# smehra34/Video-Stylization-with-NCA

Hardware: AMD Instinct MI355X
Metric: NCA cell-updates/sec (B*H*W*steps/s) at 256^2 C=16 (higher is better)
Workload: dtype f32; 1 GPU; BASELINE configs[1]: ConditionedNCA grow loop, B=8 C=16 256x256, 64 NCA steps per bench step, fp32 forward; B_per_gpu=8, C=16, H=256, W=256, nca_steps_per_bench_step=64, hidden=64, mask_rng=in-kernel philox4x32-10, parallelism=pool-shard x1 (no data-path collective)

## Files before the change

### video-stylization-with-nca_amd/csrc/nca_capi.hip

```cpp
#include "../../include/ncahip.h"

#include <cstdarg>
#include <cstdio>

#include "nca_kernels.h"

namespace {

constexpr int kMaxC = 16, kMaxCCondFwd = 32, kMaxCCondFwdBf16 = 20, kMaxCDynca = 32, kMaxFc = 128, kMaxFcFwd = 1024, kMaxHidden = 64, kMaxCond = 4;

thread_local char g_err[512] = "";

int fail(int code, const char* fmt, ...) {
    va_list ap;
    va_start(ap, fmt);
    vsnprintf(g_err, sizeof(g_err), fmt, ap);
    va_end(ap);
    return code;
}

int hip_result(hipError_t e, const char* what) {
    if (e == hipSuccess) return 0;
    snprintf(g_err, sizeof(g_err), "%s: %s", what, hipGetErrorString(e));
    return (int)e;
// ... 52 lines not shown
    std::atomic<int> state{0};
    unsigned* host = nullptr;
    unsigned* dev = nullptr;
};
ErrWord g_errw[kNcaMaxDevices];
ErrWord& errw() {
    ErrWord& w = g_errw[nca_device_index()];
    if (w.state.load(std::memory_order_acquire) == 0) {
        static std::atomic_flag lock = ATOMIC_FLAG_INIT;
        while (lock.test_and_set(std::memory_order_acquire)) {}
        if (w.state.load(std::memory_order_relaxed) == 0) {
            void *h = nullptr, *d = nullptr;
            int st = 2;
            if (hipHostMalloc(&h, 64, hipHostMallocMapped) == hipSuccess && hipHostGetDevicePointer(&d, h, 0) == hipSuccess) {
                *(volatile unsigned*)h = 0u;
                w.host = (unsigned*)h;
                w.dev = (unsigned*)d;
                st = 1;
            }
            w.state.store(st, std::memory_order_release);
        }
        lock.clear(std::memory_order_release);
    }
    return w;
}
}
unsigned* nca_error_word_device() { return errw().dev; }
unsigned nca_error_word_read(bool clear) {
    ErrWord& w = errw();
    if (!w.host) return 0u;
    const unsigned v = *(volatile unsigned*)w.host;
    if (clear && v) *(volatile unsigned*)w.host = 0u;
    return v;
}
static int device_error_rc(const char* where) {
    const unsigned v = nca_error_word_read(false);
    if (!v) return 0;
    return fail(NCAHIP_EDEVICE, "%s: a device-side failure was recorded earlier on this device (error word 0x%x: bit 0 = "
                "producer/consumer hand-off poll expired, bit 1 = neighbour poll of a persistent DyNCA / ConditionedNCA kernel expired); results since "
                "the last ncahip_check_errors are not valid", where, v);
}

extern "C" {

int ncahip_check_errors(ncahip_stream_t stream, int clear) {
    hipError_t e = hipStreamSynchronize((hipStream_t)stream);
    if (e != hipSuccess) return hip_result(e, "check_errors sync");
    const unsigned v = nca_error_word_read(clear != 0);
    if (!v) return 0;
    return fail(NCAHIP_EDEVICE, "device error word 0x%x (bit 0: a producer/consumer hand-off poll expired -- the affected launch "
                "produced stale tiles; bit 1: a neighbour poll of a persistent DyNCA / ConditionedNCA kernel expired -- that launch stopped early)", v);
}

int ncahip_debug_inject_error(unsigned bits) {
    unsigned* h = errw().host;
    if (!h) return fail(NCAHIP_EINVAL, "no error word on this device");
    *(volatile unsigned*)h |= bits;
    return 0;
}

int ncahip_debug_persist_drop_tiles(int n) {
    nca_set_persist_drop_tiles(n < 0 ? 0 : n);
    return 0;
}

int ncahip_version(void) { return NCAHIP_VERSION; }
const char* ncahip_last_error(void) { return g_err; }

int ncahip_cond_precision(int mode) {
    if (mode != 0 && mode != 1) return fail(NCAHIP_EINVAL, "cond precision: 0 (exact fp32) or 1 (bf16x3)");
    nca_set_cond_precision(mode);
    return 0;
}

static int g_force_bits = 0;
int ncahip_debug_force_generic(int on) {
    g_force_bits = on;
    nca_set_force_generic((on & 1) != 0);
    nca_set_cond_variant((on >> 1) & 1);
    nca_set_bwd_bf16_exact((on & 4) != 0);
    nca_set_bwd_variant((on & 8) ? 3 : 0);
    nca_set_bwd_fm_nosplit((on & 16) != 0);
    nca_set_cond_pc_dense((on & 32) != 0);
    return 0;
}

int ncahip_limits(int* max_c, int* max_fc, int* max_hidden) {
    if (max_c) *max_c = kMaxC;
    if (max_fc) *max_fc = kMaxFc;
    if (max_hidden) *max_hidden = kMaxHidden;
    return 0;
}

int ncahip_selftest(void* scratch, ncahip_stream_t stream) {
    if (!scratch) return fail(NCAHIP_EINVAL, "selftest: null scratch");
    hipStream_t st = (hipStream_t)stream;
    hipError_t e = hipMemsetAsync(scratch, 0, 64, st);
    if (e != hipSuccess) return hip_result(e, "selftest memset");
    e = nca_launch_selftest((int*)scratch, st);
    if (e != hipSuccess) return hip_result(e, "selftest launch");
    int host = 0;
    e = hipMemcpyAsync(&host, scratch, sizeof(int), hipMemcpyDeviceToHost, st);
    if (e == hipSuccess) e = hipStreamSynchronize(st);
    if (e != hipSuccess) return hip_result(e, "selftest sync");
    return host == 1 ? 0 : fail(NCAHIP_ERANGE, "selftest: MFMA 16x16x4 f32 lane map differs from the one assumed");
}

int ncahip_dynca_perceive_f32(const float* x, float* y, int B, int C, int H, int W, int pad_mode,
                              ncahip_stream_t stream) {
    if (!x || !y || x == y) return fail(NCAHIP_EINVAL, "dynca_perceive: null or aliased pointer");
    if (!dims_ok(B, C, H, W) || pad_mode < 0 || pad_mode > 3) return fail(NCAHIP_EINVAL, "dynca_perceive: bad argument");
    if (pad_mode == NCAHIP_PAD_REFLECT && (H < 2 || W < 2)) return fail(NCAHIP_EINVAL, "reflect pad needs H,W >= 2");
    return hip_result(nca_launch_dynca_perceive(x, y, B, C, H, W, pad_mode, (hipStream_t)stream), "dynca_perceive");
}

int ncahip_cond_perceive_f32(const float* z, const float* wp, float* y, int B, int C, int H, int W,
                             ncahip_stream_t stream) {
    if (!z || !wp || !y || z == y) return fail(NCAHIP_EINVAL, "cond_perceive: null or aliased pointer");
    if (!dims_ok(B, C, H, W)) return fail(NCAHIP_EINVAL, "cond_perceive: bad size");
    return hip_result(nca_launch_cond_perceive(z, wp, y, B, C, H, W, (hipStream_t)stream), "cond_perceive");
}

int ncahip_dynca_step_fwd_f32(const float* x_in, float* x_out, const float* cond, const float* u, const float* w1,
                              const float* b1, const float* w2, const float* b2, int B, int C, int H, int W, int fc,
                              int c_cond, int pad_mode, float update_rate, uint64_t seed, uint64_t step,
                              ncahip_stream_t stream) {
    if (int rc = check_dynca(x_in, x_out, cond, w1, b1, w2, b2, B, C, H, W, fc, c_cond, pad_mode, kMaxFcFwd)) return rc;
    if (int rc = check_bits(u_is_bits(u, seed), B, H, W, update_rate, true)) return rc;
    NcaDyncaArgs a{x_in, x_out, cond, u, w1, b1, w2, b2, B, C, H, W, fc, c_cond, pad_mode, update_rate, seed, step};
    a.u_bits = u_is_bits(u, seed);
    return hip_result(nca_launch_dynca_step_fwd(a, (hipStream_t)stream), "dynca_step_fwd");
}

int ncahip_dynca_nsteps_fwd_f32(float* states, int ring, int T, const float* cond, const float* u, const float* w1,
                                const float* b1, const float* w2, const float* b2, int B, int C, int H, int W, int fc,
                                int c_cond, int pad_mode, float update_rate, uint64_t seed, uint64_t step0,
                                ncahip_stream_t stream) {
    if (ring < 2 || T < 0) return fail(NCAHIP_EINVAL, "dynca nsteps: ring >= 2 and T >= 0 required");
    if (int rc = check_dynca(states, states + 1, cond, w1, b1, w2, b2, B, C, H, W, fc, c_cond, pad_mode, kMaxFcFwd)) return rc;
    const bool ubits = u_is_bits(u, seed);
    if (int rc = check_bits(ubits, B, H, W, update_rate, true)) return rc;
    const size_t slot = (size_t)B * C * H * W, uslot = (size_t)B * H * W;
    for (int t = 0; t < T; ++t) {
        NcaDyncaArgs a{states + (size_t)(t % ring) * slot, states + (size_t)((t + 1) % ring) * slot, cond,
                       u_at(u, ubits, t, uslot), w1, b1, w2, b2, B, C, H, W, fc, c_cond, pad_mode,
                       update_rate, seed, step0 + (uint64_t)t};
        a.u_bits = ubits;
        if (int rc = hip_result(nca_launch_dynca_step_fwd(a, (hipStream_t)stream), "dynca_nsteps_fwd")) return rc;
    }
    return 0;
}

size_t ncahip_dynca_nsteps_persist_workspace(int B, int C, int H, int W, int fc, int c_cond) {
    if (!dims_ok(B, C, H, W) || !nca_dynca_persist_shape_ok(B, C, H, W, fc, c_cond)) return 0;
    return 256 + align256((size_t)2 * nca_dynca_persist_tiles(B, H, W) * C * 108 * sizeof(unsigned long long));
}

static int dynca_persist_impl(bool two_scale, const float* x_in, float* x_out, int T, const float* cond, const float* u, const float* w1,
                                        const float* b1, const float* w2, const float* b2, int B, int C, int H, int W, int fc, int c_cond,
                                        int pad_mode, float update_rate, uint64_t seed, uint64_t step0, void* workspace,
                                        size_t workspace_bytes, unsigned epoch, ncahip_stream_t stream) {
    if (T < 1 || !workspace) return fail(NCAHIP_EINVAL, "dynca nsteps persist: T >= 1 and a workspace required");
    if (epoch < 1 || epoch >= (1u << 20)) return fail(NCAHIP_EINVAL, "dynca nsteps persist: epoch must be in [1, 2^20) (zero the workspace and restart at 1 when it runs out)");
    if (int rc = check_dynca(x_in, x_out, cond, w1, b1, w2, b2, B, C, H, W, fc, c_cond, pad_mode)) return rc;
    const size_t need = ncahip_dynca_nsteps_persist_workspace(B, C, H, W, fc, c_cond);
    if (need == 0 || T >= 4096)
// ... 705 lines not shown
```

### video-stylization-with-nca_amd/csrc/nca_cond_pc.hip

```cpp
#include "nca_cond_tile.h"

namespace {

#ifndef NCA_WT_STORE
#define NCA_WT_STORE 1
#endif
constexpr bool kNtStore = NCA_WT_STORE != 0;

template <int CP>
struct PCfg {
    using F = WCfg<CP>;
    static constexpr bool WIDE = CP > 16;
    static constexpr int XR_ROWS = WIDE ? CP : 16 * F::M3T;
    static constexpr int SZ_Z = CP * CS, SZ_XR = XR_ROWS * XRS, SZ_MK = WTH * WTW;
    static constexpr int BUF = SZ_Z + SZ_XR + SZ_MK;
    static constexpr int SCR_A3 = 0;
    static constexpr int SCR_LIFE = SCR_A3 + (WTH + 6) * RS;
    static constexpr int SCR_A2 = SCR_LIFE + (WTH + 4) * RS;
    static constexpr int SCR_FLAG = SCR_A2 + (WTH + 4) * RS;
    static constexpr int SCR = SCR_FLAG + 4;
    static constexpr int PAIR = 2 * BUF + SCR;
    static constexpr int ALIAS_END = F::OFF_W3;
    static constexpr int W_BUF0 = F::SHARED;
    static constexpr int W_SCR = W_BUF0 + 4 * BUF;
    static constexpr int W_XR1P1 = W_SCR + 4 * SCR;
    static constexpr int W_BUF1 = W_XR1P1 + SZ_XR;
    static constexpr int LDS_FLOATS = WIDE ? W_BUF1 + 2 * BUF : F::SHARED + 4 * PAIR;
    static_assert(!WIDE || BUF + SZ_Z + SZ_MK <= ALIAS_END, "pair 0's second buffer + pair 1's second Z / MK fit on the dead images");
    static_assert(BUF % 4 == 0 && SCR % 4 == 0 && SZ_Z % 4 == 0 && SZ_XR % 4 == 0 && F::SHARED % 4 == 0, "16-byte carve");
    static_assert(LDS_FLOATS * 4 <= 160 * 1024, "LDS budget");
    struct Offs { int z, xr, mk, scr; };
    static __device__ __forceinline__ Offs offs(int pair, int which) {
        if constexpr (!WIDE) {
            const int b = F::SHARED + pair * PAIR + which * BUF;
            return Offs{b, b + SZ_Z, b + SZ_Z + SZ_XR, F::SHARED + pair * PAIR + 2 * BUF};
        } else {
            const int scr = W_SCR + pair * SCR;
            if (which == 0) {
                const int b = W_BUF0 + pair * BUF;
                return Offs{b, b + SZ_Z, b + SZ_Z + SZ_XR, scr};
            }
            if (pair == 0) return Offs{0, SZ_Z, SZ_Z + SZ_XR, scr};
            if (pair == 1) return Offs{BUF, W_XR1P1, BUF + SZ_Z, scr};
            const int b = W_BUF1 + (pair - 2) * BUF;
            return Offs{b, b + SZ_Z, b + SZ_Z + SZ_XR, scr};
        }
    }
};

template <int CP, bool EXACT, typename ST, bool SPLIT = false, bool FC = false>
__global__ __launch_bounds__(kThreadsW, 2) void cond_step_fwd_pc_kernel(const NcaCondArgs a) {
    static_assert(!SPLIT || ST::BYTES == 4, "bf16x3 emulation is an option of the fp32-storage kernel");
    static_assert(!FC || (ST::BYTES == 4 && !SPLIT), "firing-cell lists: the exact-f32 fp32-storage consumer");
    constexpr bool BF = ST::BYTES == 2;
    using K = WCfg<CP>;
    using PK = PCfg<CP>;
    extern __shared__ __attribute__((aligned(16))) float smem[];
    const int tid = threadIdx.x, lane = tid & 63;
    const int wave = __builtin_amdgcn_readfirstlane(tid >> 6);
    const int C = EXACT ? CP : a.C, H = a.H, W = a.W, hid = EXACT ? 64 : a.hidden, K1 = 3 * C;
    const bool producer = wave >= 4;
    const int pair = wave & 3;
    NCA_KSTAMP(0);

    if (!producer) {
        FillRegs<4 * K::K1S4 * 256, 256> f1;
        FillRegs<4 * 16 * 64, 256> f2;
        FillRegs<K::M3T * 16 * 64, 256> f3;
        FillRegs<K::HID, 256> fb1, fb2;
        FillRegs<CP * K::WPS, 256> fwp;
        {
            fill_load(f1, a.w1, tid, [&](int idx) -> long {
                const int j = idx & 3, l = (idx >> 2) & 63, q = (idx >> 8) % K::K1S4, m = (idx >> 8) / K::K1S4;
                const int s = 4 * q + j, gg = l >> 4, o = 16 * m + (l & 15);
                const int ch = 4 * (s / 3) + gg, f = s % 3;
                return (s < K::K1S && ch < C && o < hid) ? (long)o * K1 + 3 * ch + f : -1;
            });
            fill_load(f2, a.w2, tid, [&](int idx) -> long {
                const int r = idx & 3, l = (idx >> 2) & 63, m = (idx >> 8) & 3, m2 = idx >> 10;
                const int gg = l >> 4, o = 16 * m2 + (l & 15), k = 16 * m + 4 * gg + r;
                return (o < hid && k < hid) ? (long)o * hid + k : -1;
            });
            fill_load(f3, a.w3, tid, [&](int idx) -> long {
                const int r = idx & 3, l = (idx >> 2) & 63, m = (idx >> 8) & 3, m3 = idx >> 10;
                const int gg = l >> 4, o = 16 * m3 + (l & 15), k = 16 * m + 4 * gg + r;
                return (o < C && k < hid) ? (long)o * hid + k : -1;
            });
        }
        fill_load(fb1, a.b1, tid, [&](int idx) -> long { return idx < hid ? idx : -1; });
        fill_load(fb2, a.b2, tid, [&](int idx) -> long { return idx < hid ? idx : -1; });
        fill_load(fwp, a.wp, tid, [&](int idx) -> long {
            const int ch = idx / K::WPS, j = idx % K::WPS;
            return (ch < C && j < 27) ? (long)ch * 27 + j : -1;
        });
        {
            fill_store(f1, smem + K::OFF_W1, tid);
            fill_store(f2, smem + K::OFF_W2, tid);
            fill_store(f3, smem + K::OFF_W3, tid);
        }
        fill_store(fb1, smem + K::OFF_B1, tid);
        fill_store(fb2, smem + K::OFF_B2, tid);
        fill_store(fwp, smem + K::OFF_WP, tid);
    }

    auto lds_of = [&](int which) -> TileLds {
        const typename PK::Offs o = PK::offs(pair, which);
        float* const S = smem + o.scr;
        return TileLds{smem + o.z, smem + o.xr, S + PK::SCR_A3, S + PK::SCR_A3, S + PK::SCR_LIFE, S + PK::SCR_A2, smem + o.mk,
                       reinterpret_cast<int*>(S + PK::SCR_FLAG) + 2 + which};
    };

    constexpr int PSTH = 16, PSTW = 16;
    const int st_x = (W + PSTW - 1) / PSTW, st_y = (H + PSTH - 1) / PSTH;
    const int halo = a.alive_ch >= 0 ? 3 : 1;
    NcaTileWalk tw = nca_tile_walk(a.B * st_x * st_y);
    struct Pos { int k, r, t, sx, sy, b; };
    const int n_rounds = (tw.end - tw.base + tw.stride - 1) / tw.stride;
    auto pos_first = [&]() -> Pos {
        Pos p{0, tw.local, tw.base + tw.local, 0, 0, 0};
        p.sx = p.t % st_x;
        const int q = p.t / st_x;
        p.sy = q % st_y;
        p.b = q / st_y;
        return p;
    };
    auto advance = [&](Pos p) -> Pos {
        ++p.k;
        int delta = tw.stride + 1;
        if (++p.r == tw.stride) { p.r = 0; delta = 1; }
        p.t += delta;
        p.sx += delta;
        while (p.sx >= st_x) {
            p.sx -= st_x;
            if (++p.sy == st_y) { p.sy = 0; ++p.b; }
        }
        return p;
    };
    auto tile_of = [&](const Pos& p) -> WTile {
        WTile w{0, 0, 0, false, false};
        if (p.k < n_rounds && p.t < tw.end) {
            w.b = p.b;
            w.ty0 = p.sy * PSTH + pair * WTH;
            w.tx0 = p.sx * PSTW;
            w.valid = w.ty0 < H && w.tx0 < W;
            w.inner = w.ty0 >= halo && w.ty0 + WTH + halo <= H && w.tx0 >= halo && w.tx0 + WTW + halo <= W;
        }
        return w;
    };
    int tile_no = 0;
    auto produce = [&](const WTile& t, int which) {
        if (!t.valid) return;
        TileRegs<CP, ST> R;
        const TileLds L = lds_of(which);
        if (t.inner) {
            issue_loads<CP, true, true, 0, EXACT, ST>(a, t, lane, R);
            stage_tile<CP, false, EXACT, ST, true, FC>(a, t, L, lane, R, tile_no);
        } else {
            issue_loads<CP, true, true, 1, EXACT, ST>(a, t, lane, R);
            stage_tile<CP, true, EXACT, ST, true, FC>(a, t, L, lane, R, tile_no);
        }
    };
    MlpRegs<CP> Wr;
    MlpRegsBf<CP> Wb;
    MlpRegsSplit<CP> Ws;
    auto consume = [&](const WTile& t, int which) {
        if (!t.valid) return;
        const TileLds L = lds_of(which);
        if constexpr (FC) {
            const int* const FL = reinterpret_cast<const int*>(L.MK);
            const int ng = (__builtin_amdgcn_readfirstlane(*L.NF) + 15) >> 4;
            auto cells = [&](auto nt, int gi) {
                constexpr int NTC = decltype(nt)::value;
                int zc[NTC], xc[NTC];
#pragma unroll
                for (int n = 0; n < NTC; ++n) {
                    const int e = FL[16 * (gi + n) + (lane & 15)];
                    zc[n] = e & 0xFFFF;
                    xc[n] = e >> 16;
                }
                float P[NTC][K::K1S];
                if (gi == 0) NCA_STAMP(4);
                perceive_cells_pipe<CP, NTC>(smem, L.Z, lane, zc, P);
                if (gi == 0) NCA_STAMP(5);
                mlp_cells_regs<CP, NTC>(Wr, smem, L.XR, lane, xc, P);
                if (gi == 0) NCA_STAMP(6);
            };
            int gi = 0;
#pragma unroll 1
            for (; gi + 2 <= ng; gi += 2) cells(std::integral_constant<int, 2>{}, gi);
            if (gi < ng) cells(std::integral_constant<int, 1>{}, gi);
        } else {
            constexpr int NT = 2;
#pragma unroll 1
            for (int pass = 0; pass < WTH / NT; ++pass) {
                float P[NT][K::K1S];
                if (pass == 0) NCA_STAMP(4);
#ifdef NCA_STAMPS
                if (a.seed == 0xD1A8ull || a.seed == 0xD1AAull || a.seed == 0xD1ADull) {
#pragma unroll
                    for (int n = 0; n < NT; ++n)
#pragma unroll
                        for (int s_ = 0; s_ < K::K1S; ++s_) P[n][s_] = L.Z[lane + n];
                } else
#endif
                perceive_tile_pipe<CP, NT>(smem, L.Z, lane, pass * NT, P);
                if (pass == 0) NCA_STAMP(5);
#ifdef NCA_STAMPS
                if (a.seed == 0xD1A9ull || a.seed == 0xD1ABull || a.seed == 0xD1ADull) {
                    float acc_ = 0.0f;
#pragma unroll
                    for (int n = 0; n < NT; ++n)
#pragma unroll
                        for (int s_ = 0; s_ < K::K1S; ++s_) acc_ += P[n][s_];
                    L.XR[lane] = acc_;
                } else
#endif
                if constexpr (SPLIT) mlp_tile_split<CP, NT>(Ws, smem + K::OFF_B1, smem + K::OFF_B2, L.XR, L.MK, lane, pass * NT, P);
                else if constexpr (BF) mlp_tile_bf16<CP, NT>(Wb, smem + K::OFF_B1, smem + K::OFF_B2, L.XR, L.MK, lane, pass * NT, P);
                else mlp_tile_regs<CP, NT>(Wr, smem, L.XR, L.MK, lane, pass * NT, P);
                if (pass == 0) NCA_STAMP(6);
            }
        }
        NCA_STAMP(7);
#ifdef NCA_STAMPS
        if (a.seed == 0xD1ACull || a.seed == 0xD1ADull || a.seed == 0xD1AEull) return;
#endif
        if (t.inner) store_tile<CP, false, EXACT, kNtStore && !BF, ST>(a, t, L.XR, lane);
        else store_tile<CP, true, EXACT, kNtStore && !BF, ST>(a, t, L.XR, lane);
        NCA_STAMP(8);
    };

    int which = 0;
    Pos pos = pos_first();
    WTile cur = tile_of(pos);
    int* const flags = reinterpret_cast<int*>(smem + PK::offs(pair, 0).scr + PK::SCR_FLAG);
    auto post = [&](int idx, int round) {
        wave_sync();
        __builtin_amdgcn_s_waitcnt(0xC07F);
        if (lane == 0) __hip_atomic_store(flags + idx, round, __ATOMIC_RELEASE, __HIP_MEMORY_SCOPE_WORKGROUP);
    };
    auto await = [&](int idx, int round) {
        int spins = 0;
        while (__hip_atomic_load(flags + idx, __ATOMIC_ACQUIRE, __HIP_MEMORY_SCOPE_WORKGROUP) < round && ++spins < (1 << 20))
            __builtin_amdgcn_s_sleep(1);
        if (spins >= (1 << 20) && lane == 0 && a.err) __hip_atomic_fetch_or(a.err, 1u, __ATOMIC_RELAXED, __HIP_MEMORY_SCOPE_SYSTEM);
        wave_sync();
    };
    if (producer) {
        if (lane == 0) { flags[0] = -1; flags[1] = -1; }
        __builtin_amdgcn_s_setprio(3);
        produce(cur, 0);
        post(0, 0);
        NCA_KSTAMP(1);
        __syncthreads();
        if constexpr (PK::WIDE) __syncthreads();
        NCA_KSTAMP(2);
        while (pos.k + 1 < n_rounds) {
            const Pos pn = advance(pos);
            const WTile nxt = tile_of(pn);
            __builtin_amdgcn_s_setprio(0);
            await(1, pn.k - 2);
            __builtin_amdgcn_s_setprio(3);
#ifdef NCA_STAMPS
            if (a.seed != 0xD1A6ull && (a.seed < 0xD1AAull || a.seed > 0xD1ADull))
#endif
            produce(nxt, which ^ 1);
            post(0, pn.k);
            cur = nxt;
            pos = pn;
            which ^= 1;
            ++tile_no;
        }
        NCA_KSTAMP(3);
    } else {
        NCA_KSTAMP(1);
        __syncthreads();
        NCA_KSTAMP(2);
        if constexpr (SPLIT) load_weights_split_lds<CP>(smem, lane, Ws);
        else if constexpr (BF) load_weights_bf16_lds<CP>(smem, lane, Wb);
        else mlp_load_regs<CP>(smem, lane, Wr);
        if constexpr (PK::WIDE) {
            static_assert(!PK::WIDE || !SPLIT, "wide carve: the exact-f32 and the bf16 consumer");
            __builtin_amdgcn_s_waitcnt(0xC07F);
            __syncthreads();
        }
        while (pos.k < n_rounds) {
            const Pos pn = advance(pos);
            const WTile nxt = tile_of(pn);
            await(0, pos.k);
            if (tile_no == 2) NCA_KSTAMP(4);
#ifdef NCA_STAMPS
            if (a.seed != 0xD1A7ull)
#endif
            consume(cur, which);
            if (tile_no == 2) NCA_KSTAMP(5);
            post(1, pos.k);
            if (tile_no == 2) NCA_KSTAMP(6);
            if (tile_no == 3) NCA_KSTAMP(7);
            cur = nxt;
            pos = pn;
            which ^= 1;
            ++tile_no;
        }
        NCA_KSTAMP(3);
    }
}

template <int CP, bool EXACT, typename ST = StF32, bool SPLIT = false, bool FC = false>
hipError_t launch_cond_pc(const NcaCondArgs& a, hipStream_t st) {
    using PK = PCfg<CP>;
    auto kern = cond_step_fwd_pc_kernel<CP, EXACT, ST, SPLIT, FC>;
    const size_t lds = (size_t)PK::LDS_FLOATS * sizeof(float);
    static NcaLdsAttr attr;
    if (hipError_t e = attr.ensure(reinterpret_cast<const void*>(kern), lds); e != hipSuccess) return e;
    const int cus = nca_cu_count();
    const int nst = a.B * ((a.W + 15) / 16) * ((a.H + 15) / 16);
    hipLaunchKernelGGL(kern, dim3(nst < cus ? nst : cus), dim3(kThreadsW), lds, st, a);
    return hipGetLastError();
}

bool g_pc_dense = false;
template <int CP, bool EXACT>
hipError_t launch_cond_pc_f32(const NcaCondArgs& a, hipStream_t st) {
    return g_pc_dense ? launch_cond_pc<CP, EXACT, StF32, false, false>(a, st) : launch_cond_pc<CP, EXACT, StF32, false, true>(a, st);
}

}

void nca_set_cond_pc_dense(bool on) { g_pc_dense = on; }

extern "C" void nca_debug_set_stamp_buffer_pc(void* p);
static unsigned long long* g_stamp_pc = nullptr;
extern "C" void nca_debug_set_stamp_buffer_pc(void* p) { g_stamp_pc = (unsigned long long*)p; }
#if defined(NCA_STAMPS)
unsigned long long* nca_debug_stamp_ptr() { return g_stamp_pc; }
#endif
static int g_cond_precision = 0;
void nca_set_cond_precision(int mode) { g_cond_precision = mode; }
int nca_get_cond_precision() { return g_cond_precision; }
hipError_t nca_launch_cond_step_fwd_pc(const NcaCondArgs& a_in, hipStream_t st) {
    NcaCondArgs a = a_in;
    a.dbg = g_stamp_pc;
    a.err = nca_error_word_device();
    const bool h64 = a.hidden == 64;
    if (g_cond_precision == 1 && h64) {
        if (a.C == 12) return launch_cond_pc<12, true, StF32, true>(a, st);
        if (a.C == 16) return launch_cond_pc<16, true, StF32, true>(a, st);
    }
    if (a.C == 12 && h64) return launch_cond_pc_f32<12, true>(a, st);
    if (a.C == 16 && h64) return launch_cond_pc_f32<16, true>(a, st);
    if (a.C <= 12) return launch_cond_pc_f32<12, false>(a, st);
    if (a.C <= 16) return launch_cond_pc_f32<16, false>(a, st);
    if (a.C == 20 && h64) return launch_cond_pc_f32<20, true>(a, st);
    if (a.C <= 20) return launch_cond_pc_f32<20, false>(a, st);
    return hipErrorInvalidValue;
}

hipError_t nca_launch_cond_step_fwd_bf16(const NcaCondArgs& a_in, hipStream_t st) {
    NcaCondArgs a = a_in;
    a.dbg = g_stamp_pc;
    a.err = nca_error_word_device();
    const bool h64 = a.hidden == 64;
    if (a.C == 12 && h64) return launch_cond_pc<12, true, StBF16>(a, st);
    if (a.C == 16 && h64) return launch_cond_pc<16, true, StBF16>(a, st);
    if (a.C <= 12) return launch_cond_pc<12, false, StBF16>(a, st);
    if (a.C <= 16) return launch_cond_pc<16, false, StBF16>(a, st);
    if (a.C == 20 && h64) return launch_cond_pc<20, true, StBF16>(a, st);
    if (a.C <= 20) return launch_cond_pc<20, false, StBF16>(a, st);
    return hipErrorInvalidValue;
}
```

### video-stylization-with-nca_amd/csrc/nca_cond_tile.h

```cpp
#pragma once
#include "nca_common.h"
#include "nca_kernels.h"

namespace {


constexpr int kWaves = 8, kThreadsW = kWaves * 64;
constexpr int WTH = 4, WTW = 16;
constexpr int STH = 16, STW = 32;
constexpr int RS = 24;
constexpr int ZROWS = WTH + 2, CS = ZROWS * RS;
constexpr int XRS = 68;
static_assert(CS % 32 == 16 && (4 * XRS) % 32 == 16, "bank layout");

template <int CP>
struct WCfg {
    static constexpr int HID = 64;
    static constexpr int K1S = 3 * CP / 4;
    static constexpr int K1S4 = (K1S + 3) / 4;
    static constexpr int M3T = (CP + 15) / 16;
    static constexpr int WPS = 28;
    static constexpr int OFF_W1 = 0;
    static constexpr int OFF_W2 = OFF_W1 + 4 * K1S4 * 4 * 64;
    static constexpr int OFF_W3 = OFF_W2 + 4 * 16 * 64;
// ... 33 lines not shown
            __builtin_amdgcn_sched_barrier(0);                                                         \
            asm volatile("s_memtime %0\n\ts_waitcnt lgkmcnt(0)" : "=s"(t_)::"memory");                 \
            __builtin_amdgcn_sched_barrier(0);                                                         \
            if (lane == 0) a.dbg[((size_t)(blockIdx.x * kWaves + (threadIdx.x >> 6)) * kStampTiles + tile_no) * 16 + (i)] = t_; \
        }                                                                                              \
    } while (0)
#else
#define NCA_STAMP(i) do { } while (0)
#endif

typedef float f32x2 __attribute__((ext_vector_type(2)));
__device__ __forceinline__ float wclamp(float v, float lo, float hi) { return __builtin_amdgcn_fmed3f(v, lo, hi); }
__device__ __forceinline__ f32x4 ld4(const float* p) { return *reinterpret_cast<const f32x4*>(p); }
__device__ __forceinline__ void st4(float* p, f32x4 v) { *reinterpret_cast<f32x4*>(p) = v; }
__device__ __forceinline__ float max3x3(const float* p) {
    float m = fmaxf(fmaxf(p[-RS - 1], p[-RS]), p[-RS + 1]);
    m = fmaxf(m, fmaxf(fmaxf(p[-1], p[0]), p[1]));
    return fmaxf(m, fmaxf(fmaxf(p[RS - 1], p[RS]), p[RS + 1]));
}
__device__ __forceinline__ void wave_sync() {
    __builtin_amdgcn_fence(__ATOMIC_RELEASE, "wavefront");
    __builtin_amdgcn_wave_barrier();
    __builtin_amdgcn_fence(__ATOMIC_ACQUIRE, "wavefront");
}

template <int N, int NTHR = kThreadsW, typename MapT>
__device__ __forceinline__ void fill_image_w(float* __restrict__ dst, const float* __restrict__ src, int tid, MapT map) {
    constexpr int U = 8;
    constexpr int kThreadsW = NTHR;
    for (int base = tid; base < N; base += kThreadsW * U) {
        float v[U];
        bool ok[U];
#pragma unroll
        for (int u = 0; u < U; ++u) {
            const int idx = base + kThreadsW * u;
            const long o = idx < N ? map(idx) : -1;
            ok[u] = o >= 0;
            v[u] = src[ok[u] ? o : 0];
        }
#pragma unroll
        for (int u = 0; u < U; ++u) {
            const int idx = base + kThreadsW * u;
            if (idx < N) dst[idx] = ok[u] ? v[u] : 0.0f;
        }
    }
}

template <int N, int NTHR>
struct FillRegs {
    static constexpr int PER = (N + NTHR - 1) / NTHR;
    static_assert(PER <= 32, "one mask word");
    float v[PER];
    unsigned ok;
};
template <int N, int NTHR, typename MapT>
__device__ __forceinline__ void fill_load(FillRegs<N, NTHR>& r, const float* __restrict__ src, int tid, MapT map) {
    r.ok = 0u;
#pragma unroll
    for (int u = 0; u < FillRegs<N, NTHR>::PER; ++u) {
        const int idx = tid + NTHR * u;
        const long o = idx < N ? map(idx) : -1;
        r.ok |= (o >= 0 ? 1u : 0u) << u;
        r.v[u] = src[o >= 0 ? o : 0];
    }
}
template <int N, int NTHR>
__device__ __forceinline__ void fill_store(const FillRegs<N, NTHR>& r, float* __restrict__ dst, int tid) {
#pragma unroll
    for (int u = 0; u < FillRegs<N, NTHR>::PER; ++u) {
        const int idx = tid + NTHR * u;
        if (idx < N) dst[idx] = ((r.ok >> u) & 1u) ? r.v[u] : 0.0f;
    }
}

struct TileLds {
    float* Z;
    float* XR;
    float* A3;
    float* PN;
    float* LIFE;
    float* A2;
    float* MK;
    int* NF;
};
constexpr int kFirePad = WTH * WTW << 16;
template <int CP>
__device__ __forceinline__ TileLds wave_private_lds(float* PWR) {
    using K = WCfg<CP>;
    return TileLds{PWR + K::PW_Z, PWR + K::PW_XR, PWR + K::PW_A3, PWR + K::PW_A3, PWR + K::PW_LIFE, PWR + K::PW_A2,
                   PWR + K::PW_A3 + ZROWS * RS};
}

struct WTile {
    int b, ty0, tx0;
    bool valid, inner;
};

typedef unsigned u32x4 __attribute__((ext_vector_type(4)));
typedef unsigned u32x2 __attribute__((ext_vector_type(2)));
typedef __bf16 bf16x2 __attribute__((ext_vector_type(2)));
struct StF32 {
    static constexpr int BYTES = 4;
    typedef float raw1;
    typedef f32x4 raw4;
    static __device__ __forceinline__ float cv1(raw1 v) { return v; }
    static __device__ __forceinline__ f32x4 cv4(raw4 v) { return v; }
    template <int AUX>
    static __device__ __forceinline__ raw1 ld1(__amdgpu_buffer_rsrc_t r, unsigned voff, unsigned soff) {
        return __uint_as_float(__builtin_amdgcn_raw_buffer_load_b32(r, (int)voff, (int)soff, AUX));
    }
    template <int AUX>
    static __device__ __forceinline__ raw4 ld4(__amdgpu_buffer_rsrc_t r, unsigned voff, unsigned soff) {
        return __builtin_bit_cast(f32x4, __builtin_amdgcn_raw_buffer_load_b128(r, (int)voff, (int)soff, AUX));
    }
    template <int AUX>
    static __device__ __forceinline__ void st4(__amdgpu_buffer_rsrc_t r, unsigned voff, unsigned soff, f32x4 v) {
        __builtin_amdgcn_raw_buffer_store_b128(__builtin_bit_cast(u32x4, v), r, (int)voff, (int)soff, AUX);
    }
    static __device__ __forceinline__ raw1 gld1(const void* base, unsigned elem) { return static_cast<const float*>(base)[elem]; }
    static __device__ __forceinline__ raw4 gld4(const void* base, unsigned elem) {
        return *reinterpret_cast<const f32x4*>(static_cast<const float*>(base) + elem);
    }
};
struct StBF16 {
    static constexpr int BYTES = 2;
    typedef unsigned raw1;
    typedef u32x2 raw4;
    static __device__ __forceinline__ float cv1(raw1 v) { return __uint_as_float(v << 16); }
    static __device__ __forceinline__ f32x4 cv4(raw4 v) {
        return f32x4{__uint_as_float(v[0] << 16), __uint_as_float(v[0] & 0xffff0000u), __uint_as_float(v[1] << 16),
                     __uint_as_float(v[1] & 0xffff0000u)};
    }
    template <int AUX>
    static __device__ __forceinline__ raw1 ld1(__amdgpu_buffer_rsrc_t r, unsigned voff, unsigned soff) {
        return (unsigned)__builtin_amdgcn_raw_buffer_load_b16(r, (int)voff, (int)soff, AUX);
    }
    template <int AUX>
    static __device__ __forceinline__ raw4 ld4(__amdgpu_buffer_rsrc_t r, unsigned voff, unsigned soff) {
        return __builtin_bit_cast(u32x2, __builtin_amdgcn_raw_buffer_load_b64(r, (int)voff, (int)soff, AUX));
    }
    static __device__ __forceinline__ unsigned pk2(float lo, float hi) {
        typedef float f2 __attribute__((ext_vector_type(2)));
        return __builtin_bit_cast(unsigned, __builtin_convertvector(f2{lo, hi}, bf16x2));
    }
    template <int AUX>
    static __device__ __forceinline__ void st4(__amdgpu_buffer_rsrc_t r, unsigned voff, unsigned soff, f32x4 v) {
        __builtin_amdgcn_raw_buffer_store_b64(u32x2{pk2(v[0], v[1]), pk2(v[2], v[3])}, r, (int)voff, (int)soff, AUX);
    }
    static __device__ __forceinline__ raw1 gld1(const void* base, unsigned elem) { return (unsigned)static_cast<const uint16_t*>(base)[elem]; }
    static __device__ __forceinline__ raw4 gld4(const void* base, unsigned elem) {
        return *reinterpret_cast<const u32x2*>(static_cast<const uint16_t*>(base) + elem);
    }
};
__device__ __forceinline__ unsigned nca_mul_u32(unsigned a, unsigned b) { return a * b; }
__device__ __forceinline__ __amdgpu_buffer_rsrc_t nca_rsrc(const void* base) {
    return __builtin_amdgcn_make_buffer_rsrc(const_cast<void*>(base), 0, -1, 0x00020000);
}

template <int CP, typename ST = StF32>
struct TileRegs {
    typename ST::raw1 a3v[5];
    unsigned prv[4];
    float uu, up;
    typename ST::raw4 xf[CP / 2], gf[CP / 2];
    typename ST::raw1 xh[CP / 4], gh[CP / 4];
};
// ... 106 lines not shown
    float* const Z = L.Z;
    float* const XR = L.XR;
    float* const A3 = L.A3;
    float* const PN = L.PN;
    float* const LIFE = L.LIFE;
    float* const A2 = L.A2;
    float* const MK = L.MK;

    const int C = EXACT ? CP : a.C, H = a.H, W = a.W;
    const unsigned plane = (unsigned)(H * W);
    const int gch0 = C - a.goal_ch, ty0 = t.ty0, tx0 = t.tx0;
    const bool pending = a.pre_in != nullptr, use_alive = a.alive_ch >= 0, has_goal = a.goal_ch > 0;
    int lane = lane_in;
    asm volatile("" : "+v"(lane));
    const int hl = (lane >> 5) & 1, l5 = lane & 31, q4 = (lane >> 4) & 3, ci = lane & 15;

    NCA_STAMP(8);
    wave_sync();
    bool l2ok[4];
#pragma unroll
    for (int k = 0; k < 4; ++k) {
        const int gy = ty0 - 2 + 2 * k + hl, gx = tx0 - 2 + l5;
        l2ok[k] = l5 < 20 && (!CHECK || (gy >= 0 && gy < H && gx >= 0 && gx < W));
    }
    if (use_alive) {
#pragma unroll
        for (int k = 0; k < 5; ++k) {
            const int gy = ty0 - 3 + 2 * k + hl, gx = tx0 - 3 + l5;
            const bool ok = !CHECK || (gy >= 0 && gy < H && gx >= 0 && gx < W);
            if (l5 < 22) A3[(2 * k + hl) * RS + l5 + 1] = ok ? ST::cv1(R.a3v[k]) : NCA_NEG_INF;
        }
        wave_sync();
        NCA_STAMP(9);
#pragma unroll
        for (int k = 0; k < 4; ++k) {
            const int r = 2 * k + hl;
            const float* const ac = A3 + (r + 1) * RS + l5 + 2;
            float life = 0.0f, av = NCA_NEG_INF;
            if (l2ok[k]) {
                life = 1.0f;
                av = ac[0];
                if (pending) {
                    life = (R.prv[k] != 0u && max3x3(ac) > a.thr) ? 1.0f : 0.0f;
                    av = wclamp(av * life, a.lo, a.hi);
                }
            }
            if (l5 < 20) {
                LIFE[r * RS + l5 + 2] = life;
                A2[r * RS + l5 + 2] = av;
            }
        }
        wave_sync();
    } else {
#pragma unroll
        for (int k = 0; k < 4; ++k)
            if (l5 < 20) LIFE[(2 * k + hl) * RS + l5 + 2] = l2ok[k] ? 1.0f : 0.0f;
    }
    NCA_STAMP(10);
#pragma unroll
    for (int k = 0; k < 3; ++k) {
        const int r = 2 * k + hl;
        const int gy = ty0 - 1 + r, gx = tx0 - 1 + l5;
        const bool in = l5 < 18 && (!CHECK || (gy >= 0 && gy < H && gx >= 0 && gx < W));
        float pn = 0.0f;
        if (in) pn = (!use_alive || max3x3(A2 + (r + 1) * RS + l5 + 3) > a.thr) ? 1.0f : 0.0f;
        if (l5 < 18) PN[r * RS + l5 + 3] = pn;
    }
    {
        const int cgy = ty0 + q4, cgx = tx0 + ci;
        const bool cin = !CHECK || (cgy < H && cgx < W);
        unsigned um = a.u ? 0xFFFFFFFFu : 0u;
        asm volatile("" : "+v"(um));
        float uf = __uint_as_float(__float_as_uint(R.up) | (__float_as_uint(R.uu) & um));
        if (a.u_bits) {
            const unsigned cellg = (unsigned)((size_t)t.b * plane) + (cin ? (unsigned)(__mul24(cgy, W) + cgx) : 0u);
            uf = ((__float_as_uint(R.uu) >> (cellg & 31u)) & 1u) ? 0.0f : 2.0f;
        }
        const bool fires = cin && wclamp(uf, 0.0f, 1.0f) < a.fire_rate;
        if constexpr (FCL) {
            const unsigned long long bal = __builtin_amdgcn_ballot_w64(fires);
            const int pre = (int)__builtin_amdgcn_mbcnt_hi((unsigned)(bal >> 32), __builtin_amdgcn_mbcnt_lo((unsigned)bal, 0u));
            const int cnt = __popcll(bal);
            int* const FL = reinterpret_cast<int*>(MK);
            if (fires) FL[pre] = (q4 * RS + ci) | (lane << 16);
            if (lane >= cnt) FL[lane] = kFirePad;
            if (lane == 0) *L.NF = cnt;
        } else {
            MK[lane] = fires ? 1.0f : 0.0f;
        }
        wave_sync();
        if (cin && a.pre_out)
            __builtin_amdgcn_raw_buffer_store_b8((uint8_t)PN[(q4 + 1) * RS + ci + 4], nca_rsrc(a.pre_out + (size_t)t.b * plane),
                                                 __mul24(cgy, W) + cgx, 0, kAuxCoherent);
    }
    NCA_STAMP(11);
    if (l5 < 24) {
        const int fr = l5 >> 2, ff = l5 & 3;
        const bool fok = !CHECK || (ty0 - 1 + fr >= 0 && ty0 - 1 + fr < H && tx0 + 4 * ff + 3 < W);
        const f32x4 lf = ld4(LIFE + (fr + 1) * RS + 4 + 4 * ff);
        const f32x4 pn = ld4(PN + fr * RS + 4 + 4 * ff);
        const bool inner = fr >= 1 && fr <= WTH;
        f32x4 v[CP / 2];
#pragma unroll
        for (int k = 0; k < CP / 2; ++k) {
            const int ch = 2 * k + hl;
            v[k] = ST::cv4(R.xf[k]);
            if (pending) {
                v[k] = v[k] * lf;
#pragma unroll
                for (int j = 0; j < 4; ++j) v[k][j] = wclamp(v[k][j], a.lo, a.hi);
            }
            if ((CHECK && !fok) || ch >= C) v[k] = f32x4{0.f, 0.f, 0.f, 0.f};
            if (KEEPX && inner) st4(XR + ch * XRS + (fr - 1) * WTW + 4 * ff, v[k]);
        }
        NCA_STAMP(12);
#pragma unroll
        for (int k = 0; k < CP / 2; ++k) {
            const int ch = 2 * k + hl;
            if (has_goal && ch >= gch0 && ch < C && fok) v[k] = __builtin_elementwise_fma(ST::cv4(R.gf[k]), pn, v[k]);
            st4(Z + ch * CS + fr * RS + 4 + 4 * ff, v[k]);
        }
    }
    NCA_STAMP(13);
    if (ci < 12) {
        const int hr = ci >> 1, zq = (ci & 1) ? WTW + 4 : 3;
        const int hgy = ty0 - 1 + hr, hgx = (ci & 1) ? tx0 + WTW : tx0 - 1;
        const bool hok = !CHECK || (hgy >= 0 && hgy < H && hgx >= 0 && hgx < W);
        const float lf = LIFE[(hr + 1) * RS + zq], pn = PN[hr * RS + zq];
#pragma unroll
        for (int k = 0; k < CP / 4; ++k) {
            const int ch = 4 * k + q4;
            float v = ST::cv1(R.xh[k]);
            if (pending) v = wclamp(v * lf, a.lo, a.hi);
            if (!hok || ch >= C) v = 0.0f;
            else if (has_goal && ch >= gch0) v = fmaf(ST::cv1(R.gh[k]), pn, v);
            Z[ch * CS + hr * RS + zq] = v;
        }
    }
    wave_sync();
}

template <int CP, int NT>
__device__ __forceinline__ void perceive_tile(const float* __restrict__ WS, const float* __restrict__ Z, int lane_in,
                                              int n0, float (&P)[NT][3 * CP / 4]) {
    using K = WCfg<CP>;
    int lane = lane_in;
    asm volatile("" : "+v"(lane));
    const float* const WPL = WS + K::OFF_WP;
    const int g = (lane >> 4) & 3, ci = lane & 15;
#pragma unroll
    for (int c4 = 0; c4 < CP / 4; ++c4) {
        const float* const zc = Z + (4 * c4 + g) * CS + n0 * RS + ci + 3;
        float wt[28];
#pragma unroll
        for (int j4 = 0; j4 < 7; ++j4) {
            const f32x4 w4 = ld4(WPL + (4 * c4 + g) * K::WPS + 4 * j4);
            wt[4 * j4 + 0] = w4[0]; wt[4 * j4 + 1] = w4[1]; wt[4 * j4 + 2] = w4[2]; wt[4 * j4 + 3] = w4[3];
        }
        static_assert(NT == 2, "row pairs: one v_pk_fma_f32 serves output rows n0 and n0+1");
        const unsigned za = (unsigned)(size_t)(const __attribute__((address_space(3))) float*)zc;
        f32x2 nb[9];
#define NCA_RD2(i, o) asm volatile("ds_read2_b32 %0, %1 offset0:%2 offset1:%3" : "=v"(nb[i]) : "v"(za), "n"(o), "n"((o) + RS))
        NCA_RD2(0, 0); NCA_RD2(1, 1); NCA_RD2(2, 2);
        NCA_RD2(3, RS); NCA_RD2(4, RS + 1); NCA_RD2(5, RS + 2);
        NCA_RD2(6, 2 * RS); NCA_RD2(7, 2 * RS + 1); NCA_RD2(8, 2 * RS + 2);
#undef NCA_RD2
        asm volatile("s_waitcnt lgkmcnt(0)"
                     : "+v"(nb[0]), "+v"(nb[1]), "+v"(nb[2]), "+v"(nb[3]), "+v"(nb[4]), "+v"(nb[5]), "+v"(nb[6]), "+v"(nb[7]), "+v"(nb[8])
// ... 618 lines not shown
```

### video-stylization-with-nca_amd/csrc/nca_kernels.h

```cpp
#pragma once
#include <hip/hip_runtime.h>
#include <stdint.h>

#include <atomic>

constexpr int kNcaMaxDevices = 64;
inline int nca_device_index() {
    int d = 0;
    if (hipGetDevice(&d) != hipSuccess || d < 0 || d >= kNcaMaxDevices) d = 0;
    return d;
}
inline int nca_cu_count() {
    static std::atomic<int> cus[kNcaMaxDevices];
    const int d = nca_device_index();
    int v = cus[d].load(std::memory_order_relaxed);
    if (v == 0) {
        int q = 0;
        v = 256;
        if (hipDeviceGetAttribute(&q, hipDeviceAttributeMultiprocessorCount, d) == hipSuccess && q > 0) v = q;
        cus[d].store(v, std::memory_order_relaxed);
    }
    return v;
}
struct NcaLdsAttr {
// ... 4 lines not shown
        hipError_t e = hipFuncSetAttribute(kern, hipFuncAttributeMaxDynamicSharedMemorySize, (int)bytes);
        if (e == hipSuccess) done[d].store(true, std::memory_order_release);
        return e;
    }
};
unsigned* nca_error_word_device();
unsigned nca_error_word_read(bool clear);

struct NcaDyncaArgs {
    const float* x_in;
    float* x_out;
    const float* cond;
    const float* u;
    const float *w1, *b1, *w2, *b2;
    int B, C, H, W, fc, c_cond, pad_mode;
    float rate;
    uint64_t seed, step;
    const float* g_next;
    float* hbuf;
    float* dhbuf;
    float* dybuf;
    float* g_out;
    int w2_ld;
    float* gw2_ws;
    const float* g_extra;
    const float* pc;
    const float* coarse_add;
    int dy_half;
    float* ybuf;
    int u_bits;
};

struct NcaDyncaPersistArgs {
    const float* x_in;
    float* x_out;
    int T;
    const float* cond;
    const float* u;
    const float *w1, *b1, *w2, *b2;
    int B, C, H, W, fc, c_cond, pad_mode;
    float rate;
    uint64_t seed, step0;
    int* flags;
    unsigned epoch;
    unsigned long long* xch;
    size_t xch_words;
    unsigned* err;
    int u_bits;
    int dbg;
};
void nca_set_persist_drop_tiles(int n);
bool nca_dynca_persist_shape_ok(int B, int C, int H, int W, int fc, int c_cond);
int nca_dynca_persist_tiles(int B, int H, int W);
hipError_t nca_launch_dynca_persist(const NcaDyncaPersistArgs& a, hipStream_t st, bool query_only, bool* fits);
hipError_t nca_launch_dynca_persist_ms(const NcaDyncaPersistArgs& a, hipStream_t st, bool query_only, bool* fits);

struct NcaCondPersistArgs {
    const float* x0;
    float* states;
    uint8_t* pre;
    int hist;
    float* x_final;
    const float* goal;
    const float* u;
    const float *wp, *w1, *b1, *w2, *b2, *w3;
    int B, C, H, W, goal_ch, alive_ch, T;
    float thr, fire_rate, lo, hi;
    uint64_t seed, step0;
    int* abort_w;
    unsigned epoch;
    unsigned long long* xch;
    size_t xch_words;
    unsigned* err;
    int u_bits;
    uint64_t poll_ticks;
    unsigned long long* dbg;
};
bool nca_cond_persist_shape_ok(int B, int C, int H, int W, int hidden, int goal_ch);
int nca_cond_persist_tiles(int B, int H, int W);
size_t nca_cond_persist_xch_pairs(int B, int C, int H, int W);
hipError_t nca_launch_cond_persist(const NcaCondPersistArgs& a, hipStream_t st, bool query_only, bool* fits);
int nca_get_cond_precision();
void nca_set_cond_pc_dense(bool on);
bool nca_cond_default_family();

struct NcaCondArgs {
    const float* x_in;
    const uint8_t* pre_in;
    float* x_out;
    uint8_t* pre_out;
    const float* goal;
    const float* u;
    const float *wp, *w1, *b1, *w2, *b2, *w3;
    int B, C, H, W, hidden, goal_ch, alive_ch;
    float thr, fire_rate, lo, hi;
    uint64_t seed, step;
    unsigned long long* dbg;
    unsigned* err;
    int u_bits;
};

struct NcaCondBwdArgs {
    NcaCondArgs f;
    const float* x_next;
    const uint8_t* pre_t;
    const float* g_next;
    float* g_out;
    float* gx;
    float* dP;
    float* zbuf;
    float* dgoal;
    float* slabs;
    float* wp_partials;
    int nslab, nblk;
    int srows;
    float* opimg;
    int opmode;
    int msplit;
    void* pscr;
    void* doscr;
};
int nca_cond_bwd_slab_floats(int C, int hidden);
hipError_t nca_launch_cond_bwd_unpermute(const float* red, int C, int hidden, bool bf16_history, float* g_w1, float* g_w2, float* g_w3,
                                         float* g_b1, float* g_b2, hipStream_t st);
int nca_cond_bwd_nslab();
int nca_cond_bwd_nblk(int B, int C, int H, int W);
void nca_set_bwd_fm_nosplit(bool on);
bool nca_cond_bwd_is_fm(const NcaCondBwdArgs& ba, bool bf16);
constexpr size_t kNcaCondBwdOpimgBytes = 128 * 1024;
hipError_t nca_launch_cond_step_bwd(const NcaCondBwdArgs& a, hipStream_t st, bool bf16 = false);
hipError_t nca_launch_cond_step_bwd_fm(const NcaCondBwdArgs& a, hipStream_t st, int mode);
size_t nca_cond_bwd_fm_pscr_bytes(int B, int C, int H, int W);
size_t nca_cond_bwd_fm_doscr_bytes(int B, int C, int H, int W);
void nca_set_bwd_variant(int v);
hipError_t nca_launch_reduce_rows(const float* src, float* dst, int n, int m, hipStream_t st, bool accumulate = false);
int nca_dynca_bwd_grid(int B, int H, int W);
int nca_dynca_bwd_grid_c(int B, int C, int H, int W);
int nca_gram_grid(int B, int HW);
hipError_t nca_launch_gram_rows(const float* a, int ma, const float* b1, int nb1, const float* b2, int nb2, int B, int HW,
                                float* out, float* ws, hipStream_t st, bool accumulate = false);
hipError_t nca_launch_reduce_wp(const float* part, float* dst, int B, int C, int H, int W, hipStream_t st);
int nca_ot_bands(int N);
hipError_t nca_launch_ot_gather(const float* t, const float* g, const int* idx, float* x, float* y, float* xn, float* yn, int B, int c,
                                int HW, int N, hipStream_t st);
hipError_t nca_launch_ot_scatter(const float* dy, const int* idx, float* dg, int B, int c, int HW, int N, hipStream_t st);
hipError_t nca_launch_ot_remd_fwd(const float* x, const float* y, const float* xn, const float* yn, float* rmin, int* rarg, float* cmin,
                                  int* carg, float* remd, int* branch, int B, int N, int c, void* ws, hipStream_t st);
hipError_t nca_launch_ot_remd_bwd(const float* x, const float* y, const float* xn, const float* yn, const int* rarg, const int* carg,
                                  const int* branch, const float* gup, float* dy, int B, int N, int c, hipStream_t st);

hipError_t nca_launch_dynca_step_fwd(const NcaDyncaArgs& a, hipStream_t st);
hipError_t nca_launch_cond_step_fwd(const NcaCondArgs& a, hipStream_t st);
hipError_t nca_launch_dynca_step_bwd(const NcaDyncaArgs& a, hipStream_t st);
hipError_t nca_launch_dynca_step_bwd_mlp(const NcaDyncaArgs& a, hipStream_t st, bool acc);
hipError_t nca_launch_dynca_step_bwd_stencil(const NcaDyncaArgs& a, hipStream_t st);
hipError_t nca_launch_dynca_step_fwd_bf16(const NcaDyncaArgs& a, hipStream_t st);
hipError_t nca_launch_cond_step_fwd_wave(const NcaCondArgs& a, hipStream_t st);
hipError_t nca_launch_cond_step_fwd_pc(const NcaCondArgs& a, hipStream_t st);
hipError_t nca_launch_cond_step_fwd_bf16(const NcaCondArgs& a, hipStream_t st);
hipError_t nca_launch_cond_finalize_bf16(const uint16_t* x, const uint8_t* pre, uint16_t* out, int B, int C, int H, int W,
                                         int alive_ch, float thr, float lo, float hi, hipStream_t st);
void nca_set_cond_precision(int mode);
void nca_set_bwd_bf16_exact(bool on);
void nca_set_cond_variant(int v);

void nca_debug_set_stamp_buffer(unsigned long long* p);

void nca_set_force_generic(bool on);

hipError_t nca_launch_dynca_perceive(const float* x, float* y, int B, int C, int H, int W, int pad, hipStream_t st);
hipError_t nca_launch_image_encoder_front(const float* img, const float* k3, const float* k5, float* feat, int B, int ch, int H, int W,
                                          hipStream_t st);
hipError_t nca_launch_edge_extractor(const float* img, const float* k3, float* out, int B, int H, int W, int do_tanh, hipStream_t st);
hipError_t nca_launch_widen_bf16(const uint16_t* in, float* out, size_t n, hipStream_t st);
hipError_t nca_launch_dynca_ms_combine(float* y, const float* pc, int B, int C, int H, int W, hipStream_t st);
hipError_t nca_launch_dynca_ms_upT(const float* dy, float* dpc, int B, int C, int H, int W, hipStream_t st);
int nca_dynca_bwd_ms_grid(int B, int H, int W);
hipError_t nca_launch_dynca_coarse_perceive(const float* x, float* pc, int B, int C, int H, int W, int pad, hipStream_t st);
hipError_t nca_launch_cond_perceive(const float* z, const float* wp, float* y, int B, int C, int H, int W, hipStream_t st);
hipError_t nca_launch_cond_finalize(const float* x, const uint8_t* pre, float* out, int B, int C, int H, int W,
                                    int alive_ch, float thr, float lo, float hi, hipStream_t st);
hipError_t nca_launch_cond_alive(const float* x, uint8_t* out, int B, int C, int H, int W, int alive_ch, float thr,
// ... 5 lines not shown
```

Before: 7.148 billion cell-updates/s.

## Borrow next tile's firing cells to fill partial groups and issue producer loads early

The consumer wave's firing-cell loop pads the last 16-cell group. It can now borrow firing cells from the next tile's already-staged list when the producer has posted it, which needs absolute LDS offsets stored in each firing-list entry. Separately, the producer issues global loads for the next tile before waiting on the consumer's buffer release, so load latency overlaps the wait. The cost is a bounded spin on the producer flag, extra index arithmetic per cell, and more register pressure from holding tile registers across the wait.

```diff
diff --git a/video-stylization-with-nca_amd/csrc/nca_capi.hip b/video-stylization-with-nca_amd/csrc/nca_capi.hip
--- a/video-stylization-with-nca_amd/csrc/nca_capi.hip
+++ b/video-stylization-with-nca_amd/csrc/nca_capi.hip
@@ -158,6 +158,7 @@
     nca_set_bwd_variant((on & 8) ? 3 : 0);
     nca_set_bwd_fm_nosplit((on & 16) != 0);
     nca_set_cond_pc_dense((on & 32) != 0);
+    nca_set_cond_pc_noborrow((on & 64) != 0);
     return 0;
 }
 
diff --git a/video-stylization-with-nca_amd/csrc/nca_cond_pc.hip b/video-stylization-with-nca_amd/csrc/nca_cond_pc.hip
--- a/video-stylization-with-nca_amd/csrc/nca_cond_pc.hip
+++ b/video-stylization-with-nca_amd/csrc/nca_cond_pc.hip
@@ -6,6 +6,14 @@
 #define NCA_WT_STORE 1
 #endif
 constexpr bool kNtStore = NCA_WT_STORE != 0;
+#ifndef NCA_PC_EARLY_LOADS
+#define NCA_PC_EARLY_LOADS 1
+#endif
+constexpr bool kEarlyLoads = NCA_PC_EARLY_LOADS != 0;
+#ifndef NCA_FC_LOOK_SPINS
+#define NCA_FC_LOOK_SPINS 32
+#endif
+constexpr int kLookSpins = NCA_FC_LOOK_SPINS;
 
 template <int CP>
 struct PCfg {
@@ -29,6 +37,7 @@
     static_assert(!WIDE || BUF + SZ_Z + SZ_MK <= ALIAS_END, "pair 0's second buffer + pair 1's second Z / MK fit on the dead images");
     static_assert(BUF % 4 == 0 && SCR % 4 == 0 && SZ_Z % 4 == 0 && SZ_XR % 4 == 0 && F::SHARED % 4 == 0, "16-byte carve");
     static_assert(LDS_FLOATS * 4 <= 160 * 1024, "LDS budget");
+    static_assert(LDS_FLOATS <= 0x10000, "a firing-cell list entry holds two 16-bit float indices into the allocation");
     struct Offs { int z, xr, mk, scr; };
     static __device__ __forceinline__ Offs offs(int pair, int which) {
         if constexpr (!WIDE) {
@@ -107,7 +116,7 @@
         const typename PK::Offs o = PK::offs(pair, which);
         float* const S = smem + o.scr;
         return TileLds{smem + o.z, smem + o.xr, S + PK::SCR_A3, S + PK::SCR_A3, S + PK::SCR_LIFE, S + PK::SCR_A2, smem + o.mk,
-                       reinterpret_cast<int*>(S + PK::SCR_FLAG) + 2 + which};
+                       reinterpret_cast<int*>(S + PK::SCR_FLAG) + 2 + which, (unsigned)o.z | ((unsigned)o.xr << 16)};
     };
 
     constexpr int PSTH = 16, PSTW = 16;
@@ -148,47 +157,78 @@
         return w;
     };
     int tile_no = 0;
-    auto produce = [&](const WTile& t, int which) {
+    auto produce_issue = [&](const WTile& t, TileRegs<CP, ST>& R) {
         if (!t.valid) return;
-        TileRegs<CP, ST> R;
+        if (t.inner) issue_loads<CP, true, true, 0, EXACT, ST>(a, t, lane, R);
+        else issue_loads<CP, true, true, 1, EXACT, ST>(a, t, lane, R);
+    };
+    auto produce_stage = [&](const WTile& t, int which, const TileRegs<CP, ST>& R) {
+        if (!t.valid) return;
         const TileLds L = lds_of(which);
-        if (t.inner) {
-            issue_loads<CP, true, true, 0, EXACT, ST>(a, t, lane, R);
-            stage_tile<CP, false, EXACT, ST, true, FC>(a, t, L, lane, R, tile_no);
-        } else {
-            issue_loads<CP, true, true, 1, EXACT, ST>(a, t, lane, R);
-            stage_tile<CP, true, EXACT, ST, true, FC>(a, t, L, lane, R, tile_no);
-        }
+        if (t.inner) stage_tile<CP, false, EXACT, ST, true, FC>(a, t, L, lane, R, tile_no);
+        else stage_tile<CP, true, EXACT, ST, true, FC>(a, t, L, lane, R, tile_no);
     };
     MlpRegs<CP> Wr;
     MlpRegsBf<CP> Wb;
     MlpRegsSplit<CP> Ws;
-    auto consume = [&](const WTile& t, int which) {
+    int* const flags = reinterpret_cast<int*>(smem + PK::offs(pair, 0).scr + PK::SCR_FLAG);
+    int fc_done = 0;
+    auto consume = [&](const WTile& t, int which, const WTile& nxt, int nxt_round) {
         if (!t.valid) return;
         const TileLds L = lds_of(which);
         if constexpr (FC) {
             const int* const FL = reinterpret_cast<const int*>(L.MK);
-            const int ng = (__builtin_amdgcn_readfirstlane(*L.NF) + 15) >> 4;
+            const int* const FLN = reinterpret_cast<const int*>(lds_of(which ^ 1).MK);
+            const int nf = __builtin_amdgcn_readfirstlane(*L.NF);
+            const int first = fc_done;
+            const int ng = (nf - first + 15) >> 4;
+            const int pad_e = (int)(L.FLB + (unsigned)kFirePad);
+            int nb = 0;
+            auto look = [&]() {
+                const int room = first + 16 * ng - nf;
+                if (room == 0 || !nxt.valid || a.fc_noborrow) return;
+                int spins = 0;
+                while (__builtin_amdgcn_readfirstlane(__hip_atomic_load(flags + 0, __ATOMIC_ACQUIRE, __HIP_MEMORY_SCOPE_WORKGROUP)) < nxt_round) {
+                    if (++spins > kLookSpins) return;
+                    __builtin_amdgcn_s_sleep(1);
+                }
+                const int nn = __builtin_amdgcn_readfirstlane(*lds_of(which ^ 1).NF);
+                nb = room < nn ? room : nn;
+            };
             auto cells = [&](auto nt, int gi) {
                 constexpr int NTC = decltype(nt)::value;
                 int zc[NTC], xc[NTC];
 #pragma unroll
                 for (int n = 0; n < NTC; ++n) {
-                    const int e = FL[16 * (gi + n) + (lane & 15)];
+                    const int i = first + 16 * (gi + n) + (lane & 15);
+                    const int j = i - nf;
+                    int e = FL[i < WTH * WTW - 1 ? i : WTH * WTW - 1];
+                    if (j >= 0) e = pad_e;
+                    if (nb > 0) {
+                        const int en = FLN[j < 0 ? 0 : (j < WTH * WTW - 1 ? j : WTH * WTW - 1)];
+                        if (j >= 0 && j < nb) e = en;
+                    }
                     zc[n] = e & 0xFFFF;
-                    xc[n] = e >> 16;
+                    xc[n] = (int)((unsigned)e >> 16);
                 }
                 float P[NTC][K::K1S];
                 if (gi == 0) NCA_STAMP(4);
-                perceive_cells_pipe<CP, NTC>(smem, L.Z, lane, zc, P);
+                perceive_cells_pipe<CP, NTC>(smem, smem, lane, zc, P);
                 if (gi == 0) NCA_STAMP(5);
-                mlp_cells_regs<CP, NTC>(Wr, smem, L.XR, lane, xc, P);
+                mlp_cells_regs<CP, NTC>(Wr, smem, smem, lane, xc, P);
                 if (gi == 0) NCA_STAMP(6);
             };
             int gi = 0;
 #pragma unroll 1
-            for (; gi + 2 <= ng; gi += 2) cells(std::integral_constant<int, 2>{}, gi);
-            if (gi < ng) cells(std::integral_constant<int, 1>{}, gi);
+            for (; gi + 2 <= ng; gi += 2) {
+                if (gi + 2 == ng) look();
+                cells(std::integral_constant<int, 2>{}, gi);
+            }
+            if (gi < ng) {
+                look();
+                cells(std::integral_constant<int, 1>{}, gi);
+            }
+            fc_done = nb;
         } else {
             constexpr int NT = 2;
 #pragma unroll 1
@@ -233,7 +273,6 @@
     int which = 0;
     Pos pos = pos_first();
     WTile cur = tile_of(pos);
-    int* const flags = reinterpret_cast<int*>(smem + PK::offs(pair, 0).scr + PK::SCR_FLAG);
     auto post = [&](int idx, int round) {
         wave_sync();
         __builtin_amdgcn_s_waitcnt(0xC07F);
@@ -249,7 +288,11 @@
     if (producer) {
         if (lane == 0) { flags[0] = -1; flags[1] = -1; }
         __builtin_amdgcn_s_setprio(3);
-        produce(cur, 0);
+        {
+            TileRegs<CP, ST> R;
+            produce_issue(cur, R);
+            produce_stage(cur, 0, R);
+        }
         post(0, 0);
         NCA_KSTAMP(1);
         __syncthreads();
@@ -258,13 +301,18 @@
         while (pos.k + 1 < n_rounds) {
             const Pos pn = advance(pos);
             const WTile nxt = tile_of(pn);
+            TileRegs<CP, ST> R;
+#ifdef NCA_STAMPS
+            const bool idle_p = a.seed == 0xD1A6ull || (a.seed >= 0xD1AAull && a.seed <= 0xD1ADull);
+#else
+            constexpr bool idle_p = false;
+#endif
+            if (kEarlyLoads && FC && !idle_p) produce_issue(nxt, R);
             __builtin_amdgcn_s_setprio(0);
             await(1, pn.k - 2);
             __builtin_amdgcn_s_setprio(3);
-#ifdef NCA_STAMPS
-            if (a.seed != 0xD1A6ull && (a.seed < 0xD1AAull || a.seed > 0xD1ADull))
-#endif
-            produce(nxt, which ^ 1);
+            if (!(kEarlyLoads && FC) && !idle_p) produce_issue(nxt, R);
+            if (!idle_p) produce_stage(nxt, which ^ 1, R);
             post(0, pn.k);
             cur = nxt;
             pos = pn;
@@ -292,7 +340,7 @@
 #ifdef NCA_STAMPS
             if (a.seed != 0xD1A7ull)
 #endif
-            consume(cur, which);
+            consume(cur, which, nxt, pn.k);
             if (tile_no == 2) NCA_KSTAMP(5);
             post(1, pos.k);
             if (tile_no == 2) NCA_KSTAMP(6);
@@ -320,6 +368,7 @@
 }
 
 bool g_pc_dense = false;
+bool g_pc_noborrow = false;
 template <int CP, bool EXACT>
 hipError_t launch_cond_pc_f32(const NcaCondArgs& a, hipStream_t st) {
     return g_pc_dense ? launch_cond_pc<CP, EXACT, StF32, false, false>(a, st) : launch_cond_pc<CP, EXACT, StF32, false, true>(a, st);
@@ -328,6 +377,7 @@
 }
 
 void nca_set_cond_pc_dense(bool on) { g_pc_dense = on; }
+void nca_set_cond_pc_noborrow(bool on) { g_pc_noborrow = on; }
 
 extern "C" void nca_debug_set_stamp_buffer_pc(void* p);
 static unsigned long long* g_stamp_pc = nullptr;
@@ -342,6 +392,7 @@
     NcaCondArgs a = a_in;
     a.dbg = g_stamp_pc;
     a.err = nca_error_word_device();
+    a.fc_noborrow = g_pc_noborrow ? 1 : 0;
     const bool h64 = a.hidden == 64;
     if (g_cond_precision == 1 && h64) {
         if (a.C == 12) return launch_cond_pc<12, true, StF32, true>(a, st);
diff --git a/video-stylization-with-nca_amd/csrc/nca_cond_tile.h b/video-stylization-with-nca_amd/csrc/nca_cond_tile.h
--- a/video-stylization-with-nca_amd/csrc/nca_cond_tile.h
+++ b/video-stylization-with-nca_amd/csrc/nca_cond_tile.h
@@ -139,6 +139,7 @@
     float* A2;
     float* MK;
     int* NF;
+    unsigned FLB;
 };
 constexpr int kFirePad = WTH * WTW << 16;
 template <int CP>
@@ -411,8 +412,7 @@
             const int pre = (int)__builtin_amdgcn_mbcnt_hi((unsigned)(bal >> 32), __builtin_amdgcn_mbcnt_lo((unsigned)bal, 0u));
             const int cnt = __popcll(bal);
             int* const FL = reinterpret_cast<int*>(MK);
-            if (fires) FL[pre] = (q4 * RS + ci) | (lane << 16);
-            if (lane >= cnt) FL[lane] = kFirePad;
+            if (fires) FL[pre] = (int)(L.FLB + (unsigned)((q4 * RS + ci) | (lane << 16)));
             if (lane == 0) *L.NF = cnt;
         } else {
             MK[lane] = fires ? 1.0f : 0.0f;
diff --git a/video-stylization-with-nca_amd/csrc/nca_kernels.h b/video-stylization-with-nca_amd/csrc/nca_kernels.h
--- a/video-stylization-with-nca_amd/csrc/nca_kernels.h
+++ b/video-stylization-with-nca_amd/csrc/nca_kernels.h
@@ -110,6 +110,7 @@
 hipError_t nca_launch_cond_persist(const NcaCondPersistArgs& a, hipStream_t st, bool query_only, bool* fits);
 int nca_get_cond_precision();
 void nca_set_cond_pc_dense(bool on);
+void nca_set_cond_pc_noborrow(bool on);
 bool nca_cond_default_family();
 
 struct NcaCondArgs {
@@ -126,6 +127,7 @@
     unsigned long long* dbg;
     unsigned* err;
     int u_bits;
+    int fc_noborrow;
 };
 
 struct NcaCondBwdArgs {
```

After: 7.186 billion cell-updates/s (median of 6 runs). No clear change (+0.5%).
